# Gyeeta/gyeeta

Measured on AMD Instinct MI355X. Metric: events/sec ingested + p50/p99 quantile error vs reference, 1→8 MI355X, higher is better.
Workload: dtype int64; 1 GPU; C3/C4: 10000 hosts x 1000 services, raw 24-B tcp_ipv4_resp_event_t stream, uniform over services, 1 window (ingest + window close) per step; service_keys_total=10000000, multi_level_windows=0, td_pend_cap=1920, td_pend_cap_is_library_default=False, exchange=none, exchange_requested=none, exchange_fallback=False

## Files before the change

gyeeta_amd/csrc/gys_kernels.hpp:

```cpp
#pragma once

#include "gys_device.hpp"

namespace gys {

#define GYS_HUGE_VALUE_BITS 20
#define GYS_HUGE_BINS (1u << GYS_HUGE_VALUE_BITS)
#define GYS_ROW_BITS 6
#define GYS_ROW_MASK 0x3Fu
#define GYS_ROW_V6 0x20u
#define GYS_BM_WORDS 32u
#define GYS_STAGED_WORD(tresp, cli_port) ((uint64_t)(((uint32_t)(tresp) << GYS_ROW_BITS) | ((uint32_t)(cli_port) & 0x1Fu)))
#define GYS_STAGED_WORD_FAM(tresp, cli_port, v6) ((uint32_t)(((uint32_t)(tresp) << GYS_ROW_BITS) | ((v6) ? GYS_ROW_V6 : 0u) | ((uint32_t)(cli_port) & 0x1Fu)))

enum { CTR_RESP_EVENTS = 0, CTR_RESP_DROP_RANGE, CTR_RESP_DROP_NOLISTENER, CTR_CONN_EVENTS, CTR_CONN_UNKNOWN, CTR_LSTATE_RECORDS,
       CTR_LSTATE_MISSED, CTR_LSTATE_ERRORS, CTR_LSTATE_DELETED, CTR_TD_MERGES, CTR_TD_MERGE_VALUES, CTR_ACTCONN_RECORDS, CTR_ACTCONN_REMOTE_LISTEN, CTR_ACTCONN_UNKNOWN,
       CTR_CONN_NEW, CTR_CONN_CLOSED, CTR_CONN_CLOSED_NO_NOTIFY, CTR_CONN_CLI_SIDE, CTR_RESP_RUN_OVERFLOW, CTR_NUM };

__global__ void k_table_set(DevTable t, const uint64_t *kv, uint32_t n)
{
	const uint32_t i = blockIdx.x * blockDim.x + threadIdx.x;
	if (i >= n) return;
	const uint64_t key = kv[2u * i];
	uint32_t h = get_uint64_hash(key) & t.mask;
// ... 1552 lines not shown
	__shared__ uint64_t s_T[GYS_NBP];
	__shared__ uint32_t s_imin[GYS_IVL], s_imax[GYS_IVL];
	__shared__ unsigned long long s_osum[GYS_NBP];
	__shared__ uint32_t s_ocnt[GYS_NBP];
	__shared__ uint32_t s_icnt[GYS_IVL];
	__shared__ uint32_t s_ioff[GYS_IVL + 1];
	__shared__ uint32_t s_clt[GYS_IVL];
	__shared__ unsigned long long s_fa[16], s_fw[16];
	__shared__ uint32_t s_fbm[GYS_BM_WORDS];
	__shared__ int32_t s_fmm[3];
	__shared__ uint32_t s_wv[2 * (NT / 64) + 2];
	__shared__ uint64_t s_ww[NT / 64];
	const uint32_t tid = threadIdx.x, lane = tid & 63u, wave = tid >> 6;
	const uint32_t nent = *q.count;
	const bool query = q.out_sum != nullptr;

	for (uint32_t w = blockIdx.x; w < nent; w += gridDim.x) {
		const MergeEnt ent = q.list[w];
		const uint32_t m = ent.nbuf + ent.mrun;
		if (m > MAXV) continue;
		const uint32_t slot = ent.slot;
		const uint4 mt = *(const uint4 *)&p.td_meta[slot];
		const uint32_t nh = query ? ent.nbuf : (mt.y & 0xFFFFu), nw = mt.y >> 16;
		const uint32_t nwin0 = max(nh, nw);
		const uint32_t run0 = ent.off_end - ent.mrun;

		const int64_t *gs = p.td_sum + (size_t)slot * GYS_TD_NB;
		const uint32_t *gc = p.td_cnt + (size_t)slot * GYS_TD_NB;
		uint32_t c0 = 0;
		int64_t sm0 = 0;
		if (tid < GYS_TD_NB) {
			c0 = gc[tid];
			sm0 = gs[tid];
		}
		if (m == 0) {
			if (query && tid < GYS_TD_NB) {
				q.out_sum[(size_t)w * GYS_TD_NB + tid] = sm0;
				q.out_cnt[(size_t)w * GYS_TD_NB + tid] = c0;
			}
			continue;
		}
		uint32_t pos0 = 0, nc = 0;
		uint64_t e0 = 0, nold = 0;
		{
			const unsigned long long b0 = __ballot(c0 != 0);
			const unsigned long long below = lane ? (~0ull >> (64 - lane)) : 0ull;
			const uint64_t inc = wave_incl_scan_u64(c0);
			if (lane == 63u) s_ww[wave] = inc;
			if (lane == 0u) s_wv[wave] = (uint32_t)__popcll(b0);
			__syncthreads();
			uint32_t pbase = 0;
			uint64_t wbase = 0;
#pragma unroll
			for (uint32_t k = 0; k < 4u; ++k) {
				if (k < wave) {
					pbase += s_wv[k];
					wbase += s_ww[k];
				}
				nc += s_wv[k];
				nold += s_ww[k];
			}
			pos0 = pbase + (uint32_t)__popcll(b0 & below);
			e0 = wbase + inc - c0;
		}
		const uint64_t twoN = 2ull * (nold + (uint64_t)m);
		if (tid < GYS_NBP) {
			s_thr[tid] = 0xFFFFFFFFu;
			s_T[tid] = (tid >= 1u && tid < GYS_TD_NB) ? td_threshold(c_td_bnd[tid], twoN) : (tid ? ~0ull : 0ull);
			s_osum[tid] = 0;
			s_ocnt[tid] = 0;
		}
		for (uint32_t i = tid; i < GYS_IVL; i += NT) {
			s_icnt[i] = 0;
			s_imin[i] = 0xFFFFFFFFu;
			s_imax[i] = 0;
			s_clt[i] = 0;
		}
		if (tid < 16u) {
			s_fa[tid] = 0;
			s_fw[tid] = 0;
			s_fbm[tid] = 0;
			s_fbm[tid + 16u] = 0;
		}
		if (tid == 0) {
			s_fmm[0] = INT32_MAX;
			s_fmm[1] = INT32_MIN;
			s_fmm[2] = INT32_MIN;
		}
		__syncthreads();
		if (c0) {
			s_thr[pos0] = ceil_div_sum_cnt(sm0, c0);
			s_cpfx[pos0] = e0;
		}
		if (tid == 0) s_cpfx[nc] = nold;
		__syncthreads();
		{
			const uint32_t *pend = p.td_pend + (size_t)slot * p.pcap;
			int32_t lmin = INT32_MAX, lmax = INT32_MIN, wmax = INT32_MIN;
			for (uint32_t i = tid; i < m; i += NT) {
				const uint32_t word = i < ent.nbuf ? pend[i] : p.staged[run0 + (i - ent.nbuf)];
				const uint32_t uv = word >> GYS_ROW_BITS;
				uint32_t lo = 0;
#pragma unroll
				for (uint32_t step = GYS_NBP / 2; step >= 1u; step >>= 1)
					if (s_thr[lo + step - 1u] <= uv) lo += step;
				const uint32_t iv = lo + value_grid(uv);
				s_x[i] = (iv << 20) | uv;
				atomicAdd(&s_icnt[iv], 1u);
				atomicMin(&s_imin[iv], uv);
				atomicMax(&s_imax[iv], uv);
				atomicAdd(&s_clt[lo + 1], 1u);
				if (i >= nh) {
					const uint32_t b = resp_bucket((int64_t)uv);
					const unsigned long long one = GYS_PACK_ONE | (unsigned long long)uv;
					atomicAdd(&s_fa[b], one);
					lmin = min(lmin, (int32_t)uv);
					lmax = max(lmax, (int32_t)uv);
					if (i >= nwin0) {
						atomicAdd(&s_fw[b], one);
						const uint32_t r = word & GYS_ROW_MASK;
						atomicOr(&s_fbm[r >> 1], (1u << b) << ((r & 1u) * 16u));
						wmax = max(wmax, (int32_t)uv);
					}
				}
			}
			if (!query && m > nh) {
				lmin = wave_min_i32(lmin);
				lmax = wave_max_i32(lmax);
				wmax = wave_max_i32(wmax);
				if (lane == 0) {
					if (lmin != INT32_MAX) atomicMin(&s_fmm[0], lmin);
					if (lmax != INT32_MIN) atomicMax(&s_fmm[1], lmax);
					if (wmax != INT32_MIN) atomicMax(&s_fmm[2], wmax);
				}
			}
		}
		__syncthreads();
		if (wave == 0) {
			uint32_t t[5], gcl[5];
			uint32_t own = 0, gown = 0;
#pragma unroll
			for (int k = 0; k < 5; ++k) {
				t[k] = s_icnt[5u * lane + k];
				gcl[k] = s_clt[5u * lane + k];
				own += t[k];
				gown += gcl[k];
			}
			const uint32_t inc = wave_incl_scan_u32(own), ginc = wave_incl_scan_u32(gown);
			uint32_t ex = inc - own, gex = ginc - gown;
#pragma unroll
			for (int k = 0; k < 5; ++k) {
				s_ioff[5u * lane + k] = ex;
				s_icnt[5u * lane + k] = ex;
				ex += t[k];
				gex += gcl[k];
				s_clt[5u * lane + k] = gex;
			}
			if (lane == 63u) s_ioff[GYS_IVL] = inc;
		}
		__syncthreads();
		for (uint32_t i = tid; i < m; i += NT) {
			const uint32_t x = s_x[i];
			s_g[atomicAdd(&s_icnt[x >> 20], 1u)] = x;
		}
		__syncthreads();
		if (c0) {
			const uint64_t mid2 = 2ull * (e0 + (uint64_t)s_clt[pos0 + 1]) + (uint64_t)c0;
			uint32_t a = 0;
#pragma unroll
			for (uint32_t step = GYS_NBP / 2; step >= 1u; step >>= 1)
				if (mid2 >= s_T[a + step]) a += step;
			atomicAdd(&s_osum[a], (unsigned long long)sm0);
			atomicAdd(&s_ocnt[a], c0);
		}
		for (uint32_t e = tid; e < m; e += NT) {
			const uint32_t x = s_g[e];
			const uint32_t iv = x >> 20;
			uint32_t r = e;
			if (s_imin[iv] != s_imax[iv]) {
				const uint32_t gb = s_ioff[iv], ge = s_ioff[iv + 1];
				r = gb;
				for (uint32_t t = gb; t < ge; ++t) {
					const uint32_t y = s_g[t];
					r += (y < x || (y == x && t < e)) ? 1u : 0u;
				}
			}
			const uint64_t mid2 = 2ull * ((uint64_t)r + s_cpfx[iv - value_grid(x & 0xFFFFFu)]) + 1ull;
			uint32_t a = 0;
#pragma unroll
			for (uint32_t step = GYS_NBP / 2; step >= 1u; step >>= 1)
				if (mid2 >= s_T[a + step]) a += step;
			atomicAdd(&s_osum[a], (unsigned long long)(x & 0xFFFFFu));
			atomicAdd(&s_ocnt[a], 1u);
		}
		__syncthreads();
		if (tid < GYS_TD_NB) {
			int64_t *ws = query ? q.out_sum + (size_t)w * GYS_TD_NB : p.td_sum + (size_t)slot * GYS_TD_NB;
			uint32_t *wc = query ? q.out_cnt + (size_t)w * GYS_TD_NB : p.td_cnt + (size_t)slot * GYS_TD_NB;
			ws[tid] = (int64_t)s_osum[tid];
			wc[tid] = s_ocnt[tid];
		}
		if (!query) {
			const uint32_t n_all = m - nh, n_win = m > nwin0 ? m - nwin0 : 0u;
			if (tid < 16u && n_all) fold_records(p, slot, tid, mt.w != mt.z, s_fa[tid], s_fw[tid], n_all, n_win, s_fmm[1], s_fmm[2], s_fbm[tid], s_fbm[tid + 16u]);
			if (tid == 16u) {
				*(uint4 *)&p.td_meta[slot] = make_uint4(0u, 0u, mt.z, n_win ? mt.z : mt.w);
				p.td_cur[slot] = 0;
				if (n_all) {
					const int2 mm = p.td_minmax[slot];
					if (s_fmm[0] < mm.x || s_fmm[1] > mm.y) p.td_minmax[slot] = make_int2(min(mm.x, s_fmm[0]), max(mm.y, s_fmm[1]));
				}
			}
		}
		__syncthreads();
	}
}

#ifndef GYS_MB_SKIP
#define GYS_MB_SKIP 0
#endif
#define GYS_MB_EXACT 1024u
#define GYS_MB_BINS 2048u
#define GYS_MB_BPT 8u

__device__ __forceinline__ uint32_t mb_bin_clz(uint32_t v)
{
	if (v < GYS_MB_EXACT) return v;
	const uint32_t msb = 31u - (uint32_t)__clz((int)v);
	return GYS_MB_EXACT + (msb - 10u) * 64u + ((v >> (msb - 6u)) & 63u);
}

__device__ __forceinline__ uint32_t mb_bin(uint32_t v)
{
	if (v < GYS_MB_EXACT) return v;
	return (__builtin_bit_cast(uint32_t, (float)v) >> 17) - 7744u;
}

struct MergeBP {
	DigestP d;
	const MergeEnt *list;
	const uint32_t *count;
	int64_t *out_sum;
	uint32_t *out_cnt;
	MergeEnt *slow_list;
	uint32_t *slow_count;
	const double *qs;
	uint32_t nq;
	double *qout;
};

__device__ __forceinline__ double td_quantile_dev(const uint32_t *c_cnt, const unsigned long long *c_sum, const uint32_t *c_wb, uint32_t nc, uint32_t N,
						  int32_t vmin, int32_t vmax, double q)
{
	if (!N) return 0.0;
	if (q < 0.0) q = 0.0;
	if (q > 1.0) q = 1.0;
	const double t = q * (double)N;
	uint32_t lo = 0, hi = nc;
	while (lo < hi) {
		const uint32_t mid = (lo + hi) >> 1;
		if (t < (double)c_wb[mid] + (double)c_cnt[mid] * 0.5) hi = mid; else lo = mid + 1;
	}
	double res;
	if (lo < nc) {
		const double mean = (double)(int64_t)c_sum[lo] / (double)c_cnt[lo];
		const double c = (double)c_wb[lo] + (double)c_cnt[lo] * 0.5;
		if (lo == 0) {
			const double l = (double)vmin;
			res = c <= 0.0 ? mean : l + (mean - l) * (t / c);
		} else {
			const double pm = (double)(int64_t)c_sum[lo - 1] / (double)c_cnt[lo - 1];
			const double pc = (double)c_wb[lo - 1] + (double)c_cnt[lo - 1] * 0.5;
			res = pm + (mean - pm) * ((t - pc) / (c - pc));
		}
	} else {
		const double pm = (double)(int64_t)c_sum[nc - 1] / (double)c_cnt[nc - 1];
		const double pc = (double)c_wb[nc - 1] + (double)c_cnt[nc - 1] * 0.5;
		const double h = (double)vmax, span = (double)N - pc;
		res = span <= 0.0 ? h : pm + (h - pm) * ((t - pc) / span);
	}
	return floor(res + 0.5);
}

#define GYS_MB_BIG_CAP 1024u
#ifndef GYS_MB_WAVES16
#define GYS_MB_WAVES16 5
#endif
template <bool SCAN, uint32_t VPT = 4u>
__global__ __launch_bounds__(256, (VPT == 16u ? GYS_MB_WAVES16 : 8)) void k_digest_bins(MergeBP q_arg)
{
#if defined(__HIP_DEVICE_COMPILE__)
	typedef const MergeBP __attribute__((address_space(4))) *KernargP;
	KernargP q_k = (KernargP)__builtin_amdgcn_kernarg_segment_ptr();
#define GYS_MB_Q_RELOAD() asm volatile("" : "+s"(q_k))
	const MergeBP &q = *(const MergeBP *)q_k;
#else
#define GYS_MB_Q_RELOAD() (void)0
	const MergeBP &q = q_arg;
#endif
	const DigestP &p = q.d;
	static_assert(VPT == 4u || VPT == 8u || VPT == 16u || VPT == 64u, "merges of 1024 / 2048 / 4096 values; 64: up to 16 384, streamed");
	constexpr bool STREAM = VPT > 16u;
	constexpr uint32_t RV = STREAM ? 8u : VPT;
	__shared__ __align__(16) uint32_t s_bin[GYS_MB_BINS];
	constexpr uint32_t BIG_CAP = GYS_MB_BIG_CAP;
	__shared__ __align__(16) uint32_t s_big[BIG_CAP];
	__shared__ uint32_t s_thr[GYS_NBP];
	__shared__ uint32_t s_cpfx[GYS_NBP + 1];
	__shared__ uint32_t s_T[GYS_NBP];
	__shared__ unsigned long long s_osum[GYS_TD_NB];
	__shared__ uint32_t s_ocnt[GYS_TD_NB];
	__shared__ unsigned long long s_oval[GYS_TD_NB];
	__shared__ unsigned long long s_fa[16], s_fw[16];
	__shared__ uint32_t s_fbm[GYS_BM_WORDS];
	__shared__ int32_t s_fmm[3];
	__shared__ uint32_t s_wv[4], s_ws[4], s_nbig;
	__shared__ uint64_t s_ww[4];
	const uint32_t nent = SCAN ? p.nsvc : *q.count;
	const bool query = SCAN || q.out_sum != nullptr;
	uint32_t bk_first = 0, bk_chg = GYS_MB_BPT;
	if (GYS_MB_BPT * threadIdx.x < GYS_MB_EXACT) {
		bk_first = resp_bucket((int64_t)(GYS_MB_BPT * threadIdx.x));
		for (uint32_t k = GYS_MB_BPT - 1u; k >= 1u; --k)
			if (resp_bucket((int64_t)(GYS_MB_BPT * threadIdx.x + k)) != bk_first) bk_chg = k;
	}

	for (uint32_t w = blockIdx.x; w < nent; w += gridDim.x) {
		uint32_t tid = threadIdx.x;
		GYS_OPAQUE_VGPR(tid);
		GYS_MB_Q_RELOAD();
		const uint32_t lane = tid & 63u, wave = tid >> 6;
		MergeEnt ent;
		if (SCAN) ent = MergeEnt{w, min(p.td_meta[w].npend, p.pend_cap), 0u, 0u};
		else ent = q.list[w];
		const uint32_t m = ent.nbuf + ent.mrun;
		if (m > 256u * VPT) continue;
		const uint32_t slot = ent.slot;
		const uint4 mt = *(const uint4 *)&p.td_meta[slot];
		const uint32_t nh = query ? m : (mt.y & 0xFFFFu), nw = mt.y >> 16;
		const uint32_t nh_mm = SCAN ? (mt.y & 0xFFFFu) : nh;
		const uint32_t nwin0 = max(nh, nw);
		const uint32_t run0 = ent.off_end - ent.mrun;
		uint32_t c0 = 0;
		int64_t sm0 = 0;
		if (tid < GYS_TD_NB) {
			c0 = p.td_cnt[(size_t)slot * GYS_TD_NB + tid];
			sm0 = p.td_sum[(size_t)slot * GYS_TD_NB + tid];
		}
		uint32_t wd[RV];
		const uint32_t *const pend = p.td_pend + (size_t)slot * p.pcap;
		{
#pragma unroll
			for (uint32_t k = 0; k < RV; ++k) {
				const uint32_t i = tid + 256u * k;
				wd[k] = 0;
				if (i < m) wd[k] = i < ent.nbuf ? pend[i] : p.staged[run0 + (i - ent.nbuf)];
			}
		}
		if (GYS_MB_SKIP & 32) {
			uint32_t x = c0 ^ (uint32_t)sm0;
#pragma unroll
			for (uint32_t k = 0; k < RV; ++k) x ^= wd[k];
			if (x == 0xDEADBEEFu) p.td_cur[slot] = 1;
			continue;
		}
		if (m == 0 && !SCAN) {
			if (query && tid < GYS_TD_NB) {
				q.out_sum[(size_t)w * GYS_TD_NB + tid] = sm0;
				q.out_cnt[(size_t)w * GYS_TD_NB + tid] = c0;
			}
			continue;
		}
#pragma unroll
		for (uint32_t k = 0; k < GYS_MB_BPT; ++k) s_bin[tid + 256u * k] = 0;
		s_thr[tid] = 0xFFFFFFFFu;
		if (tid < GYS_TD_NB) {
			s_osum[tid] = 0;
			s_ocnt[tid] = 0;
			s_oval[tid] = 0;
		}
		if (tid < 16u) {
			s_fa[tid] = 0;
			s_fw[tid] = 0;
			s_fbm[tid] = 0;
			s_fbm[tid + 16u] = 0;
		}
		if (tid == 0) {
			s_fmm[0] = INT32_MAX;
			s_fmm[1] = INT32_MIN;
			s_fmm[2] = INT32_MIN;
			s_nbig = 0;
		}
		const unsigned long long b0 = __ballot(c0 != 0);
		const uint64_t inc = wave_incl_scan_u64(c0);
		if (lane == 63u) s_ww[wave] = inc;
		if (lane == 0u) s_wv[wave] = (uint32_t)__popcll(b0);
		__syncthreads();
		uint32_t pbase = 0, nc = 0;
		uint64_t wbase = 0, nold64 = 0;
#pragma unroll
		for (uint32_t k = 0; k < 4u; ++k) {
			if (k < wave) {
				pbase += s_wv[k];
				wbase += s_ww[k];
			}
			nc += s_wv[k];
			nold64 += s_ww[k];
		}
		if (nold64 + (uint64_t)m >= (1ull << 31)) {
			if (tid == 0) q.slow_list[atomicAdd(q.slow_count, 1u)] = ent;
			__syncthreads();
			continue;
		}
		if (SCAN && m == 0) {
			if (tid < GYS_TD_NB) {
				s_osum[tid] = (unsigned long long)sm0;
				s_ocnt[tid] = c0;
			}
			__syncthreads();
		} else {
		const uint32_t pos0 = pbase + (uint32_t)__popcll(b0 & (lane ? (~0ull >> (64 - lane)) : 0ull));
		const uint32_t e0 = (uint32_t)(wbase + inc - c0), nold = (uint32_t)nold64;
		const uint32_t twoN = 2u * (nold + m);
		uint32_t thr = 0;
		if (c0) {
			thr = ceil_div_sum_cnt(sm0, c0);
			s_thr[pos0] = thr;
			s_cpfx[pos0] = e0;
			atomicAdd(&s_bin[mb_bin(thr)], 1u << 16);
		}
		if (tid == 0) s_cpfx[nc] = nold;
		s_T[tid] = (tid >= 1u && tid < GYS_TD_NB) ? (uint32_t)td_threshold(c_td_bnd[tid], (uint64_t)twoN) : (tid ? 0xFFFFFFFFu : 0u);
		const bool fold_scan = !query && nh == 0u;
		int32_t lmin = INT32_MAX, lmax = INT32_MIN, wmax = INT32_MIN;
		for (uint32_t cb = 0; cb < (STREAM ? m : 1u); cb += 256u * RV) {
		if (STREAM && cb) {
#pragma unroll
			for (uint32_t k = 0; k < RV; ++k) {
				const uint32_t i = cb + tid + 256u * k;
				wd[k] = 0;
				if (i < m) wd[k] = i < ent.nbuf ? pend[i] : p.staged[run0 + (i - ent.nbuf)];
			}
		}
#pragma unroll
		for (uint32_t k = 0; k < RV; ++k) {
			const uint32_t i = cb + tid + 256u * k;
			if (!(i >= m || (GYS_MB_SKIP & 4))) {
			const uint32_t uv = wd[k] >> GYS_ROW_BITS;
			atomicAdd(&s_bin[mb_bin(uv)], 1u);
			const bool big = uv >= GYS_MB_EXACT;
			if (big) {
				const uint32_t at = atomicAdd(&s_nbig, 1u);
				if (256u * VPT <= BIG_CAP || at < BIG_CAP) s_big[at] = STREAM ? uv : ((i << 20) | uv);
			}
			if (SCAN && i >= nh_mm) {
				lmin = min(lmin, (int32_t)uv);
				lmax = max(lmax, (int32_t)uv);
			}
			if (i >= nh) {
				lmin = min(lmin, (int32_t)uv);
				lmax = max(lmax, (int32_t)uv);
				const bool win = i >= nwin0;
				if (big || !fold_scan || win) {
					const uint32_t b = resp_bucket((int64_t)uv);
					const unsigned long long one = GYS_PACK_ONE | (unsigned long long)uv;
					if (big || !fold_scan) atomicAdd(&s_fa[b], one);
					if (win) {
						atomicAdd(&s_fw[b], one);
						const uint32_t r = wd[k] & GYS_ROW_MASK;
						atomicOr(&s_fbm[r >> 1], (1u << b) << ((r & 1u) * 16u));
						wmax = max(wmax, (int32_t)uv);
					}
				}
			}
			}
		}
		}
		if ((!query && m > nh) || (SCAN && m > nh_mm)) {
			lmin = wave_min_i32(lmin);
			lmax = wave_max_i32(lmax);
			wmax = wave_max_i32(wmax);
			if (lane == 0) {
				if (lmin != INT32_MAX) atomicMin(&s_fmm[0], lmin);
				if (lmax != INT32_MIN) atomicMax(&s_fmm[1], lmax);
				if (wmax != INT32_MIN) atomicMax(&s_fmm[2], wmax);
			}
		}
		__syncthreads();
		if (256u * VPT > BIG_CAP && s_nbig > BIG_CAP) {
			if (tid == 0) q.slow_list[atomicAdd(q.slow_count, 1u)] = ent;
			__syncthreads();
			continue;
		}
		if (!(GYS_MB_SKIP & 8)) {
			uint32_t bv[GYS_MB_BPT], own = 0;
			{
				const uint4 lo4 = ((const uint4 *)s_bin)[2u * tid], hi4 = ((const uint4 *)s_bin)[2u * tid + 1u];
				bv[0] = lo4.x; bv[1] = lo4.y; bv[2] = lo4.z; bv[3] = lo4.w;
				bv[4] = hi4.x; bv[5] = hi4.y; bv[6] = hi4.z; bv[7] = hi4.w;
			}
#pragma unroll
			for (uint32_t k = 0; k < GYS_MB_BPT; ++k) own += bv[k];
			const uint32_t sc = wave_incl_scan_u32(own);
			uint32_t ne_own = 0, ne_sc = 0;
			if (GYS_MB_BPT * 64u * wave < GYS_MB_EXACT) {
#pragma unroll
				for (uint32_t k = 0; k < GYS_MB_BPT; ++k) ne_own += (bv[k] & 0xFFFFu) ? 1u : 0u;
				ne_sc = wave_incl_scan_u32(ne_own);
			}
			if (lane == 63u) {
				s_ws[wave] = sc;
				s_wv[wave] = ne_sc;
			}
			__syncthreads();
			uint32_t run = sc - own;
#pragma unroll
			for (uint32_t k = 0; k < 3u; ++k)
				if (k < wave) run += s_ws[k];
			if (GYS_MB_BPT * 64u * wave < GYS_MB_EXACT && s_nbig <= BIG_CAP / 2u) {
				uint16_t *const s_ne = (uint16_t *)(s_big + BIG_CAP / 2u);
				uint32_t at = ne_sc - ne_own;
#pragma unroll
				for (uint32_t k = 0; k < (GYS_MB_EXACT / (GYS_MB_BPT * 64u)) - 1u; ++k)
					if (k < wave) at += s_wv[k];
#pragma unroll
				for (uint32_t k = 0; k < GYS_MB_BPT; ++k)
					if (bv[k] & 0xFFFFu) s_ne[at++] = (uint16_t)(GYS_MB_BPT * tid + k);
			}
			unsigned long long acc0 = 0, acc1 = 0;
#pragma unroll
			for (uint32_t k = 0; k < GYS_MB_BPT; ++k) {
				const uint32_t bin = GYS_MB_BPT * tid + k;
				const uint32_t raw = bv[k];
				bv[k] = (run & 0xFFFFu) | (((run >> 16) + (raw >> 16)) << 16);
				run += raw;
				const uint32_t cnt = raw & 0xFFFFu;
				const unsigned long long d = ((unsigned long long)(cnt << 8) << 32) | (unsigned long long)(cnt * bin);
				if (k < bk_chg) acc0 += d; else acc1 += d;
			}
			((uint4 *)s_bin)[2u * tid] = make_uint4(bv[0], bv[1], bv[2], bv[3]);
			((uint4 *)s_bin)[2u * tid + 1u] = make_uint4(bv[4], bv[5], bv[6], bv[7]);
			if (fold_scan && GYS_MB_BPT * tid < GYS_MB_EXACT) {
				if (acc0) atomicAdd(&s_fa[bk_first], acc0);
				if (acc1) atomicAdd(&s_fa[bk_first + 1u], acc1);
			}
		}
		__syncthreads();
		const uint32_t nbig = s_nbig;
		const bool has_old = c0 && !(GYS_MB_SKIP & 2);
		if (has_old) {
			uint32_t nb = s_bin[mb_bin(thr)] & 0xFFFFu;
			if (thr >= GYS_MB_EXACT) {
				const uint32_t sh = (31u - (uint32_t)__clz((int)thr)) - 6u;
				const uint32_t lo = (thr >> sh) << sh, span = thr - lo;
				const uint32_t n4 = nbig & ~3u;
				for (uint32_t j = 0; j < n4; j += 4u) {
					const uint4 e4 = *(const uint4 *)&s_big[j];
					nb += ((e4.x & 0xFFFFFu) - lo < span ? 1u : 0u) + ((e4.y & 0xFFFFFu) - lo < span ? 1u : 0u) + ((e4.z & 0xFFFFFu) - lo < span ? 1u : 0u) +
					      ((e4.w & 0xFFFFFu) - lo < span ? 1u : 0u);
				}
				for (uint32_t j = n4; j < nbig; ++j) nb += (s_big[j] & 0xFFFFFu) - lo < span ? 1u : 0u;
			}
			const uint32_t mid2 = 2u * (e0 + nb) + c0;
			uint32_t a = 0;
#pragma unroll
			for (uint32_t step = GYS_NBP / 2; step >= 1u; step >>= 1)
				if (mid2 >= s_T[a + step]) a += step;
			atomicAdd(&s_osum[a], (unsigned long long)sm0);
			atomicAdd(&s_ocnt[a], c0);
		}
#ifndef GYS_MB_GROUP
#define GYS_MB_GROUP 1u
#endif
		constexpr uint32_t MBG = SCAN ? 1u : GYS_MB_GROUP;
		const bool compact = MBG == 1u && nbig <= BIG_CAP / 2u;
		if (compact) {
			const uint16_t *const s_ne = (const uint16_t *)(s_big + BIG_CAP / 2u);
			uint32_t n_ne = 0;
			if (!(GYS_MB_SKIP & (1 | 8))) {
#pragma unroll
				for (uint32_t k = 0; k < GYS_MB_EXACT / (GYS_MB_BPT * 64u); ++k) n_ne += s_wv[k];
			}
			for (uint32_t i = tid; i < n_ne; i += 256u) {
				const uint32_t b = s_ne[i];
				const uint32_t bw = s_bin[b];
				uint32_t rem = (s_bin[b + 1u] & 0xFFFFu) - (bw & 0xFFFFu), mid2 = 2u * ((bw & 0xFFFFu) + s_cpfx[bw >> 16]) + 1u, a = 0;
#pragma unroll
				for (uint32_t step = GYS_NBP / 2; step >= 1u; step >>= 1)
					if (mid2 >= s_T[a + step]) a += step;
				while (rem) {
					const uint32_t Tn = s_T[a + 1u];
					const uint32_t kk = min(rem, (Tn - mid2 + 1u) >> 1);
					atomicAdd(&s_oval[a], ((unsigned long long)kk << 40) | (unsigned long long)(kk * b));
					rem -= kk;
					mid2 += 2u * kk;
					++a;
				}
			}
		} else
#pragma unroll
		for (uint32_t k0 = 0; k0 < GYS_MB_EXACT / 256u; k0 += MBG) {
			uint32_t bq[MBG], cq[MBG], mq[MBG], aq[MBG], call = 0;
#pragma unroll
			for (uint32_t u = 0; u < MBG; ++u) {
				bq[u] = tid + 256u * (k0 + u);
				const uint32_t bw = s_bin[bq[u]];
				cq[u] = (GYS_MB_SKIP & 1) ? 0u : (s_bin[bq[u] + 1u] & 0xFFFFu) - (bw & 0xFFFFu);
				mq[u] = 2u * ((bw & 0xFFFFu) + s_cpfx[bw >> 16]) + 1u;
				aq[u] = 0;
				call |= cq[u];
			}
			if (!call) continue;
#pragma unroll
			for (uint32_t step = GYS_NBP / 2; step >= 1u; step >>= 1) {
				uint32_t tq[MBG];
#pragma unroll
				for (uint32_t u = 0; u < MBG; ++u) tq[u] = s_T[aq[u] + step];
#pragma unroll
				for (uint32_t u = 0; u < MBG; ++u)
					if (mq[u] >= tq[u]) aq[u] += step;
			}
#pragma unroll
			for (uint32_t u = 0; u < MBG; ++u) GYS_OPAQUE_VGPR(aq[u]);
#pragma unroll
			for (uint32_t u = 0; u < MBG; ++u) {
				uint32_t rem = cq[u], mid2 = mq[u], a = aq[u];
				const uint32_t b = bq[u];
				while (rem) {
					const uint32_t Tn = s_T[a + 1u];
					const uint32_t kk = min(rem, (Tn - mid2 + 1u) >> 1);
					atomicAdd(&s_oval[a], ((unsigned long long)kk << 40) | (unsigned long long)(kk * b));
					rem -= kk;
					mid2 += 2u * kk;
					++a;
				}
			}
		}
		for (uint32_t j = tid; j < ((GYS_MB_SKIP & 2) ? 0u : nbig); j += 256u) {
			const uint32_t me = s_big[j], uv = me & 0xFFFFFu;
			const uint32_t sh = (31u - (uint32_t)__clz((int)uv)) - 6u;
			uint32_t r = s_bin[mb_bin(uv)] & 0xFFFFu;
			if (STREAM) {
				for (uint32_t jj = 0; jj < nbig; ++jj) {
					const uint32_t e = s_big[jj], u = e & 0xFFFFFu;
					r += ((u >> sh) == (uv >> sh) && (u < uv || (u == uv && jj < j))) ? 1u : 0u;
				}
			} else {
				const uint32_t base = ((uv >> sh) << sh) << 12, span = ((me << 12) | (me >> 20)) - base;
				const uint32_t n4 = nbig & ~3u;
				for (uint32_t jj = 0; jj < n4; jj += 4u) {
					const uint4 e4 = *(const uint4 *)&s_big[jj];
					r += ((((e4.x << 12) | (e4.x >> 20)) - base < span) ? 1u : 0u) + ((((e4.y << 12) | (e4.y >> 20)) - base < span) ? 1u : 0u) +
					     ((((e4.z << 12) | (e4.z >> 20)) - base < span) ? 1u : 0u) + ((((e4.w << 12) | (e4.w >> 20)) - base < span) ? 1u : 0u);
				}
				for (uint32_t jj = n4; jj < nbig; ++jj) {
					const uint32_t e = s_big[jj];
					r += (((e << 12) | (e >> 20)) - base < span) ? 1u : 0u;
				}
			}
			uint32_t gap = 0;
#pragma unroll
			for (uint32_t step = GYS_NBP / 2; step >= 1u; step >>= 1)
				if (s_thr[gap + step - 1u] <= uv) gap += step;
			const uint32_t mid2 = 2u * (r + s_cpfx[gap]) + 1u;
			uint32_t a = 0;
#pragma unroll
			for (uint32_t step = GYS_NBP / 2; step >= 1u; step >>= 1)
				if (mid2 >= s_T[a + step]) a += step;
			atomicAdd(&s_oval[a], GYS_PACK_ONE | (unsigned long long)uv);
		}
		__syncthreads();
		if (tid < GYS_TD_NB) {
			const unsigned long long pv = s_oval[tid];
			s_osum[tid] += GYS_PACK_SUM(pv);
			s_ocnt[tid] += (uint32_t)(pv >> 40);
		}
		if (SCAN) __syncthreads();
		}
		if (SCAN) {
			const uint32_t oc = tid < GYS_TD_NB ? s_ocnt[tid] : 0u;
			const unsigned long long os = tid < GYS_TD_NB ? s_osum[tid] : 0ull;
			const unsigned long long ob = __ballot(oc != 0);
			const uint32_t sc = wave_incl_scan_u32(oc);
			if (lane == 63u) s_ws[wave] = sc;
			if (lane == 0u) s_wv[wave] = (uint32_t)__popcll(ob);
			__syncthreads();
			uint32_t pb = 0, wb = 0, ncq = 0, Nq = 0;
#pragma unroll
			for (uint32_t k = 0; k < 4u; ++k) {
				if (k < wave) {
					pb += s_wv[k];
					wb += s_ws[k];
				}
				ncq += s_wv[k];
				Nq += s_ws[k];
			}
			if (oc) {
				const uint32_t pos = pb + (uint32_t)__popcll(ob & (lane ? (~0ull >> (64 - lane)) : 0ull));
				s_thr[pos] = oc;
				s_cpfx[pos] = wb + sc - oc;
				s_osum[pos] = os;
			}
			__syncthreads();
			if (tid < q.nq) {
				const int2 mm = p.td_minmax[slot];
				q.qout[(size_t)slot * q.nq + tid] = td_quantile_dev(s_thr, s_osum, s_cpfx, ncq, Nq, min(mm.x, s_fmm[0]), max(mm.y, s_fmm[1]), q.qs[tid]);
			}
			__syncthreads();
			continue;
		}
		if (GYS_MB_SKIP & 16) {
			if (tid == 208u && !query) {
				*(uint4 *)&p.td_meta[slot] = make_uint4(0u, 0u, mt.z, mt.w);
				p.td_cur[slot] = 0;
			}
			__syncthreads();
			continue;
		}
		if (tid < GYS_TD_NB) {
			int64_t *ws = query ? q.out_sum + (size_t)w * GYS_TD_NB : p.td_sum + (size_t)slot * GYS_TD_NB;
			uint32_t *wc = query ? q.out_cnt + (size_t)w * GYS_TD_NB : p.td_cnt + (size_t)slot * GYS_TD_NB;
			ws[tid] = (int64_t)s_osum[tid];
			wc[tid] = s_ocnt[tid];
		}
		if (!query) {
			const uint32_t n_all = m - nh, n_win = m > nwin0 ? m - nwin0 : 0u;
			if (tid >= 192u && tid < 208u && n_all)
				fold_records(p, slot, tid - 192u, mt.w != mt.z, s_fa[tid - 192u], s_fw[tid - 192u], n_all, n_win, s_fmm[1], s_fmm[2], s_fbm[tid - 192u], s_fbm[tid - 176u]);
			if (tid == 208u) {
				*(uint4 *)&p.td_meta[slot] = make_uint4(0u, 0u, mt.z, n_win ? mt.z : mt.w);
				p.td_cur[slot] = 0;
				if (n_all) {
					const int2 mm = p.td_minmax[slot];
					if (s_fmm[0] < mm.x || s_fmm[1] > mm.y) p.td_minmax[slot] = make_int2(min(mm.x, s_fmm[0]), max(mm.y, s_fmm[1]));
				}
			}
		}
		__syncthreads();
	}
}

struct HugeP {
	DigestP d;
	const MergeEnt *huge_list;
	const uint32_t *huge_count;
	uint32_t *scratch;
};

__global__ __launch_bounds__(256) void k_digest_huge(HugeP p)
{
	__shared__ int64_t s_csum[GYS_TD_NB];
	__shared__ uint32_t s_ccnt[GYS_TD_NB];
	__shared__ uint64_t s_cpfx[GYS_TD_NB + 1];
	__shared__ uint64_t s_T[GYS_TD_NB + 1];
	__shared__ unsigned long long s_osum[GYS_TD_NB];
	__shared__ unsigned long long s_ocnt[GYS_TD_NB];
	__shared__ uint32_t s_part[256];
	__shared__ uint32_t s_wave[4];
	__shared__ unsigned long long s_ha[32], s_hw[32];
	__shared__ uint32_t s_bm[GYS_BM_WORDS];
	__shared__ uint32_t s_nc;
	__shared__ int32_t s_min, s_max, s_wmax;
	uint32_t *bins = p.scratch + (size_t)blockIdx.x * GYS_HUGE_BINS;
	const uint32_t nh_list = *p.huge_count;
	const uint32_t BPT = GYS_HUGE_BINS / 256u;

	for (uint32_t w = blockIdx.x; w < nh_list; w += gridDim.x) {
		const MergeEnt ent = p.huge_list[w];
		const uint32_t slot = ent.slot;
		const uint32_t m = ent.mrun, npend = ent.nbuf;
		const uint32_t start = ent.off_end - m;
		const uint4 mt = *(const uint4 *)&p.d.td_meta[slot];
		const uint32_t nh = mt.y & 0xFFFFu, nw = mt.y >> 16;
		const uint32_t nwin0 = max(nh, nw);
		const uint32_t *pend = p.d.td_pend + (size_t)slot * p.d.pcap;
		for (uint32_t i = threadIdx.x; i < GYS_HUGE_BINS / 4u; i += 256u) ((uint4 *)bins)[i] = make_uint4(0, 0, 0, 0);
		if (threadIdx.x < GYS_TD_NB) {
			s_osum[threadIdx.x] = 0;
			s_ocnt[threadIdx.x] = 0;
		}
		if (threadIdx.x < 32u) {
			s_ha[threadIdx.x] = 0;
			s_hw[threadIdx.x] = 0;
		}
		if (threadIdx.x >= 160u && threadIdx.x < 160u + GYS_BM_WORDS) s_bm[threadIdx.x - 160u] = 0;
		if (threadIdx.x == 0) {
			const int64_t *gs = p.d.td_sum + (size_t)slot * GYS_TD_NB;
			const uint32_t *gc = p.d.td_cnt + (size_t)slot * GYS_TD_NB;
			uint32_t nc = 0;
			uint64_t run = 0;
			for (uint32_t j = 0; j < GYS_TD_NB; ++j) {
				if (gc[j]) {
					s_csum[nc] = gs[j];
					s_ccnt[nc] = gc[j];
					s_cpfx[nc] = run;
					run += gc[j];
					nc++;
				}
			}
			s_cpfx[nc] = run;
			s_nc = nc;
			s_min = INT32_MAX;
			s_max = INT32_MIN;
			s_wmax = INT32_MIN;
		}
		__syncthreads();
		const uint32_t nc = s_nc;
		const uint64_t nold = s_cpfx[nc];
		const uint64_t twoN = 2ull * (nold + (uint64_t)m + (uint64_t)npend);
		if (threadIdx.x >= 1 && threadIdx.x < GYS_TD_NB) s_T[threadIdx.x] = td_threshold(c_td_bnd[threadIdx.x], twoN);
		if (threadIdx.x == 0) s_T[GYS_TD_NB] = ~0ull;
		{
			int32_t lmin = INT32_MAX, lmax = INT32_MIN, wmax = INT32_MIN;
			for (uint32_t i = threadIdx.x; i < npend + m; i += 256u) {
				const uint32_t word = i < npend ? pend[i] : p.d.staged[start + (i - npend)];
				const uint32_t v = (word >> GYS_ROW_BITS) & (GYS_HUGE_BINS - 1u);
				atomicAdd(&bins[v], 1u);
				if (i >= nh) {
					const uint32_t hb = resp_bucket((int64_t)v);
					atomicAdd(&s_ha[2 * hb], 1ull);
					atomicAdd(&s_ha[2 * hb + 1], (unsigned long long)v);
					lmin = min(lmin, (int32_t)v);
					lmax = max(lmax, (int32_t)v);
					if (i >= nwin0) {
						atomicAdd(&s_hw[2 * hb], 1ull);
						atomicAdd(&s_hw[2 * hb + 1], (unsigned long long)v);
						const uint32_t row = word & GYS_ROW_MASK;
						const uint32_t bit = (1u << hb) << ((row & 1u) * 16u);
						if ((s_bm[row >> 1] & bit) == 0) atomicOr(&s_bm[row >> 1], bit);
						wmax = max(wmax, (int32_t)v);
					}
				}
			}
			atomicMin(&s_min, lmin);
			atomicMax(&s_max, lmax);
			atomicMax(&s_wmax, wmax);
		}
		__syncthreads();
		__builtin_amdgcn_fence(__ATOMIC_ACQUIRE, "agent");
		uint32_t part = 0;
		{
			const uint4 *b4 = (const uint4 *)(bins + threadIdx.x * BPT);
			for (uint32_t i = 0; i < BPT / 4u; ++i) {
				const uint4 v = b4[i];
				part += v.x + v.y + v.z + v.w;
			}
		}
		uint32_t tot;
		const uint32_t pfx = block_exclusive_scan_256(part, s_wave, &tot);
		s_part[threadIdx.x] = pfx;
		__syncthreads();
		if (threadIdx.x < nc) {
			const int64_t cs = s_csum[threadIdx.x];
			const uint32_t cc = s_ccnt[threadIdx.x];
			uint64_t lt = 0;
			if (cs > 0) {
				int64_t vmax = (cs - 1) / (int64_t)cc;
				if (vmax >= (int64_t)GYS_HUGE_BINS) vmax = GYS_HUGE_BINS - 1;
				const uint32_t owner = (uint32_t)vmax / BPT;
				lt = s_part[owner];
				for (uint32_t b = owner * BPT; b <= (uint32_t)vmax; ++b) lt += bins[b];
			}
			const uint64_t mid2 = 2ull * (s_cpfx[threadIdx.x] + lt) + (uint64_t)cc;
			const uint32_t cl = td_cluster_of(s_T, mid2);
			atomicAdd(&s_osum[cl], (unsigned long long)cs);
			atomicAdd(&s_ocnt[cl], (unsigned long long)cc);
		}
		{
			uint64_t r0 = pfx;
			uint32_t ci = 0;
			const uint32_t vbeg = threadIdx.x * BPT;
			{
				uint32_t lo = 0, hi = nc;
				const int64_t v = (int64_t)vbeg;
				while (lo < hi) {
					const uint32_t mid = (lo + hi) >> 1;
					if (s_csum[mid] <= v * (int64_t)s_ccnt[mid]) lo = mid + 1; else hi = mid;
				}
				ci = lo;
			}
			for (uint32_t b = vbeg; b < vbeg + BPT; ++b) {
				const uint32_t c = bins[b];
				if (!c) continue;
				const int64_t v = (int64_t)b;
				while (ci < nc && s_csum[ci] <= v * (int64_t)s_ccnt[ci]) ci++;
				const uint64_t le = s_cpfx[ci];
				const uint64_t first = 2ull * (r0 + le) + 1ull, last = first + 2ull * (uint64_t)(c - 1u);
				uint32_t cl = td_cluster_of(s_T, first);
				const uint32_t cl_last = td_cluster_of(s_T, last);
				uint64_t rbeg = r0;
				for (; cl <= cl_last; ++cl) {
					uint64_t rend;
					if (cl == cl_last) {
						rend = r0 + c;
					} else {
						const uint64_t Tn = s_T[cl + 1];
						rend = (Tn / 2ull) - le;
						if (rend > r0 + c) rend = r0 + c;
					}
					if (rend > rbeg) {
						const uint64_t k = rend - rbeg;
						atomicAdd(&s_osum[cl], (unsigned long long)(k * (uint64_t)v));
						atomicAdd(&s_ocnt[cl], (unsigned long long)k);
						rbeg = rend;
					}
				}
				r0 += c;
			}
		}
		__syncthreads();
		if (threadIdx.x < GYS_TD_NB) {
			p.d.td_sum[(size_t)slot * GYS_TD_NB + threadIdx.x] = (int64_t)s_osum[threadIdx.x];
			p.d.td_cnt[(size_t)slot * GYS_TD_NB + threadIdx.x] = (uint32_t)s_ocnt[threadIdx.x];
		}
		{
			const uint32_t n_all = npend + m - nh, n_win = npend + m - nwin0;
			const uint32_t t = threadIdx.x - 128u;
			if (threadIdx.x >= 128u && t < 16u) {
				gys_hist_serial *ap = (gys_hist_serial *)&p.d.hist_all[slot] + t, *wp = (gys_hist_serial *)&p.d.hist_win[slot] + t;
				const bool roll = mt.w != mt.z;
				gys_hist_serial av = *ap;
				if (t < 15u) {
					av.count += s_ha[2 * t];
					av.sum += (int64_t)s_ha[2 * t + 1];
				} else {
					av.count += n_all;
					if (av.sum < (int64_t)s_max) av.sum = (int64_t)s_max;
				}
				*ap = av;
				if (n_win) {
					gys_hist_serial wv;
					if (roll) {
						wv.count = 0;
						wv.sum = t < 15u ? 0 : INT64_MIN;
					} else {
						wv = *wp;
					}
					if (t < 15u) {
						wv.count += s_hw[2 * t];
						wv.sum += (int64_t)s_hw[2 * t + 1];
					} else {
						wv.count += n_win;
						if (wv.sum < (int64_t)s_wmax) wv.sum = (int64_t)s_wmax;
					}
					*wp = wv;
					uint32_t *bp = &p.d.bitmap[(size_t)slot * GYS_BM_WORDS + t];
					*bp = (roll ? 0u : *bp) | s_bm[t];
					bp[16] = (roll ? 0u : bp[16]) | s_bm[t + 16u];
				}
			}
			__syncthreads();
			if (threadIdx.x == 0) {
				*(uint4 *)&p.d.td_meta[slot] = make_uint4(0u, 0u, mt.z, n_win ? mt.z : mt.w);
				p.d.td_cur[slot] = 0;
				const int2 mm = p.d.td_minmax[slot];
				p.d.td_minmax[slot] = make_int2(min(mm.x, s_min), max(mm.y, s_max));
			}
		}
		__syncthreads();
	}
// ... 1699 lines not shown
```

Measured before the change: 71.50 billion events/s.

## Bucket-group big values in digest merge and add lean fold-scan ingest path

```diff
diff --git a/gyeeta_amd/csrc/gys_kernels.hpp b/gyeeta_amd/csrc/gys_kernels.hpp
--- a/gyeeta_amd/csrc/gys_kernels.hpp
+++ b/gyeeta_amd/csrc/gys_kernels.hpp
@@ -1878,6 +1878,8 @@
 	static_assert(VPT == 4u || VPT == 8u || VPT == 16u || VPT == 64u, "merges of 1024 / 2048 / 4096 values; 64: up to 16 384, streamed");
 	constexpr bool STREAM = VPT > 16u;
 	constexpr uint32_t RV = STREAM ? 8u : VPT;
+	constexpr bool GROUP = !STREAM;
+	constexpr uint32_t GE = GYS_MB_BIG_CAP / 256u;
 	__shared__ __align__(16) uint32_t s_bin[GYS_MB_BINS];
 	constexpr uint32_t BIG_CAP = GYS_MB_BIG_CAP;
 	__shared__ __align__(16) uint32_t s_big[BIG_CAP];
@@ -1925,14 +1927,16 @@
 		}
 		uint32_t wd[RV];
 		const uint32_t *const pend = p.td_pend + (size_t)slot * p.pcap;
-		{
-#pragma unroll
-			for (uint32_t k = 0; k < RV; ++k) {
-				const uint32_t i = tid + 256u * k;
-				wd[k] = 0;
-				if (i < m) wd[k] = i < ent.nbuf ? pend[i] : p.staged[run0 + (i - ent.nbuf)];
-			}
-		}
+		const uint32_t m_s = (uint32_t)__builtin_amdgcn_readfirstlane((int)m), nbuf_s = (uint32_t)__builtin_amdgcn_readfirstlane((int)ent.nbuf);
+		const auto load_word = [&](uint32_t base) -> uint32_t {
+			const uint32_t i = base + tid;
+			if (base + 256u <= nbuf_s) return pend[i];
+			uint32_t x = 0;
+			if (base < m_s && i < m) x = i < ent.nbuf ? pend[i] : p.staged[run0 + (i - ent.nbuf)];
+			return x;
+		};
+#pragma unroll
+		for (uint32_t k = 0; k < RV; ++k) wd[k] = load_word(256u * k);
 		if (GYS_MB_SKIP & 32) {
 			uint32_t x = c0 ^ (uint32_t)sm0;
 #pragma unroll
@@ -2007,27 +2011,43 @@
 		}
 		if (tid == 0) s_cpfx[nc] = nold;
 		s_T[tid] = (tid >= 1u && tid < GYS_TD_NB) ? (uint32_t)td_threshold(c_td_bnd[tid], (uint64_t)twoN) : (tid ? 0xFFFFFFFFu : 0u);
-		const bool fold_scan = !query && nh == 0u;
+		const bool fold_scan = !query && __builtin_amdgcn_readfirstlane((int)nh) == 0;
 		int32_t lmin = INT32_MAX, lmax = INT32_MIN, wmax = INT32_MIN;
+		const uint32_t lean_end = min(m_s, (uint32_t)__builtin_amdgcn_readfirstlane((int)nwin0));
 		for (uint32_t cb = 0; cb < (STREAM ? m : 1u); cb += 256u * RV) {
 		if (STREAM && cb) {
 #pragma unroll
-			for (uint32_t k = 0; k < RV; ++k) {
-				const uint32_t i = cb + tid + 256u * k;
-				wd[k] = 0;
-				if (i < m) wd[k] = i < ent.nbuf ? pend[i] : p.staged[run0 + (i - ent.nbuf)];
-			}
+			for (uint32_t k = 0; k < RV; ++k) wd[k] = load_word(cb + 256u * k);
 		}
 #pragma unroll
 		for (uint32_t k = 0; k < RV; ++k) {
-			const uint32_t i = cb + tid + 256u * k;
+			const uint32_t base = cb + 256u * k, i = base + tid;
+			if (base >= m_s) break;
+			if (!SCAN && fold_scan && base + 256u <= lean_end) {
+				if (!(GYS_MB_SKIP & 4)) {
+					const uint32_t uv = wd[k] >> GYS_ROW_BITS;
+					lmin = min(lmin, (int32_t)uv);
+					lmax = max(lmax, (int32_t)uv);
+					if (uv >= GYS_MB_EXACT) {
+						const uint32_t arr = atomicAdd(&s_bin[mb_bin(uv)], 1u) & 0xFFFFu;
+						const uint32_t at = atomicAdd(&s_nbig, 1u);
+						if (256u * VPT <= BIG_CAP || at < BIG_CAP) s_big[at] = STREAM ? uv : ((arr << 20) | uv);
+						atomicAdd(&s_fa[resp_bucket((int64_t)uv)], GYS_PACK_ONE | (unsigned long long)uv);
+					} else {
+						atomicAdd(&s_bin[uv], 1u);
+					}
+				}
+				continue;
+			}
 			if (!(i >= m || (GYS_MB_SKIP & 4))) {
 			const uint32_t uv = wd[k] >> GYS_ROW_BITS;
-			atomicAdd(&s_bin[mb_bin(uv)], 1u);
 			const bool big = uv >= GYS_MB_EXACT;
 			if (big) {
+				const uint32_t arr = atomicAdd(&s_bin[mb_bin(uv)], 1u) & 0xFFFFu;
 				const uint32_t at = atomicAdd(&s_nbig, 1u);
-				if (256u * VPT <= BIG_CAP || at < BIG_CAP) s_big[at] = STREAM ? uv : ((i << 20) | uv);
+				if (256u * VPT <= BIG_CAP || at < BIG_CAP) s_big[at] = STREAM ? uv : ((arr << 20) | uv);
+			} else {
+				atomicAdd(&s_bin[uv], 1u);
 			}
 			if (SCAN && i >= nh_mm) {
 				lmin = min(lmin, (int32_t)uv);
@@ -2068,6 +2088,16 @@
 			__syncthreads();
 			continue;
 		}
+		const uint32_t nbig_s = (uint32_t)__builtin_amdgcn_readfirstlane((int)s_nbig);
+		const bool grouped = GROUP && nbig_s != 0u && !(GYS_MB_SKIP & 8);
+		uint32_t ge[GE];
+#pragma unroll
+		for (uint32_t r = 0; r < GE; ++r) ge[r] = 0;
+		if (grouped) {
+#pragma unroll
+			for (uint32_t r = 0; r < GE; ++r)
+				if (256u * r < nbig_s && tid + 256u * r < nbig_s) ge[r] = s_big[tid + 256u * r];
+		}
 		if (!(GYS_MB_SKIP & 8)) {
 			uint32_t bv[GYS_MB_BPT], own = 0;
 			{
@@ -2103,30 +2133,56 @@
 				for (uint32_t k = 0; k < GYS_MB_BPT; ++k)
 					if (bv[k] & 0xFFFFu) s_ne[at++] = (uint16_t)(GYS_MB_BPT * tid + k);
 			}
-			unsigned long long acc0 = 0, acc1 = 0;
+			if (fold_scan && GYS_MB_BPT * tid < GYS_MB_EXACT) {
+				uint32_t chg = bk_chg;
+				GYS_OPAQUE_VGPR(chg);
+				const uint32_t s0 = own & 0xFFFFu;
+				uint32_t s1 = 0;
+#pragma unroll
+				for (uint32_t k = 1; k < GYS_MB_BPT; ++k) s1 += k * (bv[k] & 0xFFFFu);
+				uint32_t a0 = s0, a1 = s1;
+				if (chg < GYS_MB_BPT) {
+					a0 = 0;
+					a1 = 0;
+#pragma unroll
+					for (uint32_t k = 0; k < GYS_MB_BPT - 1u; ++k) {
+						const uint32_t c = k < chg ? (bv[k] & 0xFFFFu) : 0u;
+						a0 += c;
+						a1 += k * c;
+					}
+				}
+				const uint32_t bin0 = GYS_MB_BPT * tid, z0 = s0 - a0;
+				const unsigned long long acc0 = ((unsigned long long)(a0 << 8) << 32) | (unsigned long long)(bin0 * a0 + a1);
+				const unsigned long long acc1 = ((unsigned long long)(z0 << 8) << 32) | (unsigned long long)(bin0 * z0 + (s1 - a1));
+				if (acc0) atomicAdd(&s_fa[bk_first], acc0);
+				if (acc1) atomicAdd(&s_fa[bk_first + 1u], acc1);
+			}
 #pragma unroll
 			for (uint32_t k = 0; k < GYS_MB_BPT; ++k) {
-				const uint32_t bin = GYS_MB_BPT * tid + k;
 				const uint32_t raw = bv[k];
 				bv[k] = (run & 0xFFFFu) | (((run >> 16) + (raw >> 16)) << 16);
 				run += raw;
-				const uint32_t cnt = raw & 0xFFFFu;
-				const unsigned long long d = ((unsigned long long)(cnt << 8) << 32) | (unsigned long long)(cnt * bin);
-				if (k < bk_chg) acc0 += d; else acc1 += d;
 			}
 			((uint4 *)s_bin)[2u * tid] = make_uint4(bv[0], bv[1], bv[2], bv[3]);
 			((uint4 *)s_bin)[2u * tid + 1u] = make_uint4(bv[4], bv[5], bv[6], bv[7]);
-			if (fold_scan && GYS_MB_BPT * tid < GYS_MB_EXACT) {
-				if (acc0) atomicAdd(&s_fa[bk_first], acc0);
-				if (acc1) atomicAdd(&s_fa[bk_first + 1u], acc1);
-			}
 		}
 		__syncthreads();
 		const uint32_t nbig = s_nbig;
-		const bool has_old = c0 && !(GYS_MB_SKIP & 2);
+		const uint32_t nsmall = s_bin[GYS_MB_EXACT] & 0xFFFFu;
+		if (grouped) {
+#pragma unroll
+			for (uint32_t r = 0; r < GE; ++r)
+				if (256u * r < nbig_s && tid + 256u * r < nbig_s) s_big[(s_bin[mb_bin(ge[r] & 0xFFFFFu)] & 0xFFFFu) - nsmall + (ge[r] >> 20)] = ge[r];
+			__syncthreads();
+		}
+		const bool has_old = c0 && !(GYS_MB_SKIP & (2 | 64));
 		if (has_old) {
 			uint32_t nb = s_bin[mb_bin(thr)] & 0xFFFFu;
 			if (thr >= GYS_MB_EXACT) {
+				if (GROUP) {
+					const uint32_t st = nb - nsmall, cn = (s_bin[mb_bin(thr) + 1u] & 0xFFFFu) - nb;
+					for (uint32_t j = 0; j < cn; ++j) nb += (s_big[st + j] & 0xFFFFFu) < thr ? 1u : 0u;
+				} else {
 				const uint32_t sh = (31u - (uint32_t)__clz((int)thr)) - 6u;
 				const uint32_t lo = (thr >> sh) << sh, span = thr - lo;
 				const uint32_t n4 = nbig & ~3u;
@@ -2136,6 +2192,7 @@
 					      ((e4.w & 0xFFFFFu) - lo < span ? 1u : 0u);
 				}
 				for (uint32_t j = n4; j < nbig; ++j) nb += (s_big[j] & 0xFFFFFu) - lo < span ? 1u : 0u;
+				}
 			}
 			const uint32_t mid2 = 2u * (e0 + nb) + c0;
 			uint32_t a = 0;
@@ -2212,26 +2269,28 @@
 				}
 			}
 		}
-		for (uint32_t j = tid; j < ((GYS_MB_SKIP & 2) ? 0u : nbig); j += 256u) {
-			const uint32_t me = s_big[j], uv = me & 0xFFFFFu;
+		for (uint32_t j = tid; j < ((GYS_MB_SKIP & (2 | 128)) ? 0u : nbig); j += 256u) {
+			uint32_t me;
+			if (GROUP) {
+				me = ge[0];
+#pragma unroll
+				for (uint32_t r = 0; r + 1u < GE; ++r) ge[r] = ge[r + 1u];
+			} else {
+				me = s_big[j];
+			}
+			const uint32_t uv = me & 0xFFFFFu;
 			const uint32_t sh = (31u - (uint32_t)__clz((int)uv)) - 6u;
 			uint32_t r = s_bin[mb_bin(uv)] & 0xFFFFu;
-			if (STREAM) {
+			if (GROUP) {
+				const uint32_t st = r - nsmall, cn = (s_bin[mb_bin(uv) + 1u] & 0xFFFFu) - r, key = (me << 12) | (me >> 20);
+				for (uint32_t jj = 0; jj < cn; ++jj) {
+					const uint32_t e = s_big[st + jj];
+					r += (((e << 12) | (e >> 20)) < key) ? 1u : 0u;
+				}
+			} else {
 				for (uint32_t jj = 0; jj < nbig; ++jj) {
 					const uint32_t e = s_big[jj], u = e & 0xFFFFFu;
 					r += ((u >> sh) == (uv >> sh) && (u < uv || (u == uv && jj < j))) ? 1u : 0u;
-				}
-			} else {
-				const uint32_t base = ((uv >> sh) << sh) << 12, span = ((me << 12) | (me >> 20)) - base;
-				const uint32_t n4 = nbig & ~3u;
-				for (uint32_t jj = 0; jj < n4; jj += 4u) {
-					const uint4 e4 = *(const uint4 *)&s_big[jj];
-					r += ((((e4.x << 12) | (e4.x >> 20)) - base < span) ? 1u : 0u) + ((((e4.y << 12) | (e4.y >> 20)) - base < span) ? 1u : 0u) +
-					     ((((e4.z << 12) | (e4.z >> 20)) - base < span) ? 1u : 0u) + ((((e4.w << 12) | (e4.w >> 20)) - base < span) ? 1u : 0u);
-				}
-				for (uint32_t jj = n4; jj < nbig; ++jj) {
-					const uint32_t e = s_big[jj];
-					r += (((e << 12) | (e >> 20)) - base < span) ? 1u : 0u;
 				}
 			}
 			uint32_t gap = 0;
```

Result: faster. 77.03 billion events/s (median of 6 runs) (+7.7%).
